# chao-ji/ldm_tf2

Measured on AMD Instinct MI355X. Metric: images/sec (256x256, 200 DDIM steps, CFG=5), higher is better.
Workload: dtype bf16

## Files before the change

### include/ldm_hip.h

```cpp
#ifndef LDM_HIP_H
#define LDM_HIP_H

#include <stddef.h>
#include <stdint.h>

#ifdef __cplusplus
extern "C" {
#endif

#define LDM_F32 0
#define LDM_BF16 1

#define LDM_OK 0
#define LDM_ERR_ARG (-1)
#define LDM_ERR_LAUNCH (-2)
#define LDM_ERR_WORKSPACE (-3)

#define LDM_ACT_NONE 0
#define LDM_ACT_GELU 1
#define LDM_ACT_GEGLU 2
#define LDM_ACT_SILU 3

int ldm_version(void);
int ldm_last_error(char* buf, int n);
// ... 21 lines not shown
  float alpha;
  int32_t no_lead_pad;
  void* ln_out;
  const float* ln_gamma;
  const float* ln_beta;
  int64_t ld_ln;
  float ln_eps;
  void* out2;
  int64_t ld2, stride2;
  int32_t n_split, rows2;
  const float* ln_cs;
  int32_t defer_reduce;
  const void* a2;
  int64_t lda2;
  int32_t Cin2;
} ldm_gemm_params;

int ldm_gemm(const ldm_gemm_params* p, void* stream);
int ldm_gemm_splits(const ldm_gemm_params* p);
int ldm_gemm_reduce(const ldm_gemm_params* p, void* stream);
int ldm_groupnorm_splitk_supported(int B, int HW, int C, int groups, int dtype);
int ldm_groupnorm_splitk_form(int B, int HW, int C, int groups, int dtype, int* form);
int ldm_groupnorm_splitk(const ldm_gemm_params* p, const float* gamma, const float* beta, void* gn_out,
                         int64_t ld_gn, int B, int HW, int groups, float eps, int silu, int store_out,
                         void* stream);
int ldm_gemm_ln_supported(int N, int dtype);
int ldm_gemm_plan(const ldm_gemm_params* p, int* tile, int* split_k);
size_t ldm_gemm_workspace_bytes(const ldm_gemm_params* p);

int ldm_conv3x3_small(const void* x, int64_t ldx, int in_dtype, const float* kernel_hwio,
                      const float* bias, void* out, int64_t ldo, int out_dtype,
                      int B, int H, int W, int Cin, int Cout, void* stream);

int ldm_groupnorm_nchunks(int B, int HW, int C);
int ldm_groupnorm_partial(const void* x, int64_t ldx, float* partial, int B, int HW, int C,
                          int groups, int nchunks, int dtype, void* stream);
int ldm_groupnorm_apply(const void* x, int64_t ldx, const float* partial, const float* gamma,
                        const float* beta, void* out, int64_t ldo, int B, int HW, int C,
                        int groups, int nchunks, float eps, int silu, int dtype, void* stream);
int ldm_groupnorm_fused_supported(int B, int HW, int C, int groups, int dtype);
int ldm_groupnorm_fused_form(int B, int HW, int C, int groups, int dtype, int* form);
int ldm_groupnorm_fused(const void* x, int64_t ldx, const float* gamma, const float* beta, void* out,
                        int64_t ldo, int B, int HW, int C, int groups, float eps, int silu, int dtype,
                        void* stream);
int ldm_layernorm(const void* x, int64_t ldx, const float* gamma, const float* beta, void* out,
                  int64_t ldo, int rows, int C, float eps, int dtype, void* stream);

int ldm_softmax_rows(const void* x, int64_t ldx, int in_dtype, void* out, int64_t ldo,
                     int out_dtype, int rows, int cols, float scale, void* stream);

int ldm_attention(const void* q, int64_t ldq, int64_t q_bs, const void* k, int64_t ldk,
                  int64_t k_bs, const void* vt, int64_t ldvt, int64_t vt_bs, void* out,
                  int64_t ldo, int64_t o_bs, int batch, int heads, int Tq, int Tk, int Sp,
                  float scale, int dtype, void* stream);

int ldm_attention_ms(const void* q, int64_t ldq, int64_t q_bs, const void* k, int64_t ldk,
                     int64_t k_bs, const void* vt, int64_t ldvt, int64_t vt_bs, void* out,
                     int64_t ldo, int64_t o_bs, int batch, int heads, int Tq, int Tk, int Sp,
                     int dtype, void* stream);

int ldm_st_tail(const void* att, int64_t lda, int K0, const void* wo, const float* bo, const void* r0,
                int64_t ldr0, const void* w1, const float* aux, const void* w2, const float* b2,
                const void* wp, const float* bp, const void* r1, int64_t ldr1, void* out, int64_t ldo,
                int M, int C, float eps, int dtype, void* stream);
int ldm_st_xtail(const void* q, int64_t ldq, int K0, const void* ctx_k, const void* ctx_vt, int Tk, int ldv, int T,
                 const void* wo, const float* bo, const void* r0, int64_t ldr0, const void* w1, const float* aux,
// ... 139 lines not shown
```

### ldm_tf2_amd/_lib.py

```python
from __future__ import annotations

import ctypes as C
import os

_HERE = os.path.dirname(os.path.abspath(__file__))
LIB_PATH = os.environ.get("LDM_HIP_LIB") or os.path.join(_HERE, "lib", "libldm_hip.so")

F32, BF16 = 0, 1
ACT_NONE, ACT_GELU, ACT_GEGLU, ACT_SILU = 0, 1, 2, 3
OK, ERR_ARG, ERR_LAUNCH, ERR_WORKSPACE = 0, -1, -2, -3
RESIZE_MODES = {"nearest": 0, "bilinear": 1, "bicubic": 2}
RESAMPLE_FILTERS = ("triangle", "cubic", "lanczos3")

c_i64, c_i32, c_f32, c_vp, c_sz = C.c_int64, C.c_int32, C.c_float, C.c_void_p, C.c_size_t
c_u32 = C.c_uint32


class GemmParams(C.Structure):
  _fields_ = [
      ("a", c_vp), ("w", c_vp), ("bias", c_vp), ("addend", c_vp), ("residual", c_vp),
      ("out", c_vp), ("workspace", c_vp), ("workspace_bytes", c_sz),
      ("lda", c_i64), ("ldr", c_i64), ("ldc_m", c_i64), ("ldc_n", c_i64),
      ("stride_a", c_i64), ("stride_w", c_i64), ("stride_c", c_i64), ("stride_r", c_i64),
      ("add_ld", c_i64),
      ("M", c_i32), ("N", c_i32), ("K", c_i32), ("batch", c_i32),
      ("add_rows", c_i32),
      ("conv", c_i32), ("B", c_i32), ("H", c_i32), ("W", c_i32), ("Cin", c_i32),
      ("OH", c_i32), ("OW", c_i32), ("stride", c_i32), ("upsample", c_i32),
      ("act", c_i32), ("dtype", c_i32), ("out_dtype", c_i32), ("split_k", c_i32),
      ("tile", c_i32), ("alpha", c_f32),
      ("no_lead_pad", c_i32),
      ("ln_out", c_vp), ("ln_gamma", c_vp), ("ln_beta", c_vp), ("ld_ln", c_i64), ("ln_eps", c_f32),
      ("out2", c_vp), ("ld2", c_i64), ("stride2", c_i64), ("n_split", c_i32), ("rows2", c_i32),
      ("ln_cs", c_vp), ("defer_reduce", c_i32),
      ("a2", c_vp), ("lda2", c_i64), ("Cin2", c_i32),
  ]


SIGNATURES = {
    "ldm_version": (c_i32, []),
    "ldm_last_error": (c_i32, [C.c_char_p, c_i32]),
    "ldm_gemm": (c_i32, [C.POINTER(GemmParams), c_vp]),
    "ldm_gemm_workspace_bytes": (c_sz, [C.POINTER(GemmParams)]),
    "ldm_gemm_splits": (c_i32, [C.POINTER(GemmParams)]),
    "ldm_gemm_reduce": (c_i32, [C.POINTER(GemmParams), c_vp]),
    "ldm_groupnorm_splitk_supported": (c_i32, [c_i32, c_i32, c_i32, c_i32, c_i32]),
    "ldm_groupnorm_splitk_form": (c_i32, [c_i32, c_i32, c_i32, c_i32, c_i32, C.POINTER(c_i32)]),
    "ldm_groupnorm_splitk": (c_i32, [C.POINTER(GemmParams), c_vp, c_vp, c_vp, c_i64, c_i32, c_i32, c_i32, c_f32,
                                     c_i32, c_i32, c_vp]),
    "ldm_conv3x3_small": (c_i32, [c_vp, c_i64, c_i32, c_vp, c_vp, c_vp, c_i64, c_i32,
                                  c_i32, c_i32, c_i32, c_i32, c_i32, c_vp]),
    "ldm_groupnorm_nchunks": (c_i32, [c_i32, c_i32, c_i32]),
    "ldm_groupnorm_partial": (c_i32, [c_vp, c_i64, c_vp, c_i32, c_i32, c_i32, c_i32, c_i32,
                                      c_i32, c_vp]),
    "ldm_groupnorm_apply": (c_i32, [c_vp, c_i64, c_vp, c_vp, c_vp, c_vp, c_i64, c_i32, c_i32,
                                    c_i32, c_i32, c_i32, c_f32, c_i32, c_i32, c_vp]),
    "ldm_layernorm": (c_i32, [c_vp, c_i64, c_vp, c_vp, c_vp, c_i64, c_i32, c_i32, c_f32,
                              c_i32, c_vp]),
    "ldm_softmax_rows": (c_i32, [c_vp, c_i64, c_i32, c_vp, c_i64, c_i32, c_i32, c_i32, c_f32,
                                 c_vp]),
    "ldm_attention": (c_i32, [c_vp, c_i64, c_i64, c_vp, c_i64, c_i64, c_vp, c_i64, c_i64,
                              c_vp, c_i64, c_i64, c_i32, c_i32, c_i32, c_i32, c_i32, c_f32,
                              c_i32, c_vp]),
    "ldm_attention_ms": (c_i32, [c_vp, c_i64, c_i64, c_vp, c_i64, c_i64, c_vp, c_i64, c_i64,
                                 c_vp, c_i64, c_i64, c_i32, c_i32, c_i32, c_i32, c_i32, c_i32, c_vp]),
    "ldm_st_tail": (c_i32, [c_vp, c_i64, c_i32, c_vp, c_vp, c_vp, c_i64, c_vp, c_vp, c_vp, c_vp, c_vp, c_vp, c_vp, c_i64,
                            c_vp, c_i64, c_i32, c_i32, c_f32, c_i32, c_vp]),
    "ldm_st_xtail": (c_i32, [c_vp, c_i64, c_i32, c_vp, c_vp, c_i32, c_i32, c_i32, c_vp, c_vp, c_vp, c_i64, c_vp, c_vp, c_vp,
                             c_vp, c_vp, c_vp, c_vp, c_i64, c_vp, c_i64, c_i32, c_i32, c_f32, c_i32, c_vp]),
    "ldm_st_block": (c_i32, [c_vp, c_i64, c_i32, c_vp, c_vp, c_vp, c_i64, c_vp, c_vp, c_vp, c_vp, c_vp, c_i32, c_i32, c_i32,
                             c_vp, c_vp, c_vp, c_vp, c_vp, c_vp, c_vp, c_vp, c_vp, c_i64, c_vp, c_i64, c_i32, c_i32, c_i32,
                             c_f32, c_i32, c_vp]),
    "ldm_ffn_geglu_supported": (c_i32, [c_i32, c_i32, c_i32]),
    "ldm_ffn_geglu": (c_i32, [c_vp, c_i64, c_vp, c_vp, c_vp, c_vp, c_vp, c_i64, c_i32, c_i32, c_f32, c_i32, c_vp]),
    "ldm_time_embedding": (c_i32, [c_vp, c_vp, c_vp, c_vp, c_i32, c_i32, c_vp]),
    "ldm_select_row": (c_i32, [c_vp, c_i64, c_i32, c_i32, c_vp, c_i32, c_vp, c_vp]),
    "ldm_gemv": (c_i32, [c_vp, c_i64, c_vp, c_vp, c_vp, c_i64, c_i32, c_i32, c_i32, c_i32,
                         c_i32, c_i32, c_vp]),
    "ldm_cfg_ddim_update": (c_i32, [c_vp, c_vp, c_vp, c_i64, c_vp, c_vp, c_vp, c_i32, c_vp, c_vp, c_i32,
                                    c_f32, c_i32, c_i32, c_i64, c_vp]),
    "ldm_cfg_ddim_update_masked": (c_i32, [c_vp, c_vp, c_vp, c_i64, c_vp, c_vp, c_vp, c_i32, c_vp, c_vp, c_i32,
                                           c_f32, c_i32, c_i32, c_i64, c_vp, c_vp, c_vp, c_i64, c_vp, c_i32, c_vp]),
    "ldm_cfg_plms_update": (c_i32, [c_vp, c_vp, c_vp, c_vp, c_vp, c_vp, c_i32, c_vp, c_vp, c_vp, c_i32, c_f32, c_i32,
                                    c_i64, c_vp, c_vp, c_vp, c_i64, c_vp, c_i32, c_vp]),
# ... 74 lines not shown
```

### ldm_tf2_amd/layout.py

```python
from __future__ import annotations

import numpy as np
import torch

ATTN_SP = (32, 48, 64, 80, 96, 160)


def padded_head(s: int) -> int:
  for sp in ATTN_SP:
    if s <= sp:
      return sp
  raise ValueError(f"head size {s} > {ATTN_SP[-1]} is not supported by the fused attention kernel")


def _dev(a, dtype, device):
  t = a if isinstance(a, torch.Tensor) else torch.from_numpy(np.ascontiguousarray(a))
  return t.to(dtype).contiguous().to(device)


def conv_kernel(k_hwio, dtype, device):
  k = torch.from_numpy(np.ascontiguousarray(k_hwio))
  cout = k.shape[3]
  return _dev(k.permute(3, 0, 1, 2).reshape(cout, -1), dtype, device)


def upsample_phase_kernel(k_hwio, dtype, device):
  k = torch.from_numpy(np.ascontiguousarray(k_hwio)).to(torch.float64)
  assert k.shape[0] == 3 and k.shape[1] == 3
  cin, cout = k.shape[2], k.shape[3]
  groups = (((0,), (1, 2)), ((0, 1), (2,)))
  out = torch.empty(4, cout, 4 * cin, dtype=torch.float64)
  for a in range(2):
    for b in range(2):
      for dy in range(2):
        for dx in range(2):
          s = sum(k[kh, kw] for kh in groups[a][dy] for kw in groups[b][dx])
          t = dy * 2 + dx
          out[2 * a + b, :, t * cin:(t + 1) * cin] = s.t()
  return _dev(out, dtype, device)


def conv_shortcut_kernel(k_hwio, k_io, dtype, device):
  k = torch.from_numpy(np.ascontiguousarray(k_hwio))
  cout = k.shape[3]
  sc = torch.from_numpy(np.ascontiguousarray(k_io)).t()
  assert sc.shape[0] == cout
  return _dev(torch.cat([k.permute(3, 0, 1, 2).reshape(cout, -1), sc], 1), dtype, device)


def dense_kernel(k_io, dtype, device):
  return _dev(torch.from_numpy(np.ascontiguousarray(k_io)).t(), dtype, device)


def split_kernel(k_dhs, sp, dtype, device):
  k = torch.from_numpy(np.ascontiguousarray(k_dhs))
  d, h, s = k.shape
# ... 92 lines not shown
```

### ldm_tf2_amd/model_runners.py

```python
from __future__ import annotations

import sys

import numpy as np
import torch

from . import ops
from ._lib import LdmHipError
from .autoencoder import AutoencoderKL, AutoencoderVQ
from .resample import check_filter, crop_box


def _tf_linspace_f32(start, stop, num):
  start, stop = np.float32(start), np.float32(stop)
  delta = np.float32((stop - start) / np.float32(num - 1))
  inner = (start + delta * np.arange(1, num - 1, dtype=np.float32)).astype(np.float32)
  return np.concatenate([[start], inner, [stop]]).astype(np.float32)


def _extract(data, t):
  return np.asarray(data).astype(np.float32)[np.asarray(t)].reshape(-1, 1, 1, 1)


def normal_latents(seed, first_index, count, shape_hwc, stream=None):
# ... 356 lines not shown
PLMS_WEIGHTS = (
    (1.,),
    (3. / 2., -1. / 2.),
    (23. / 12., -16. / 12., 5. / 12.),
    (55. / 24., -59. / 24., 37. / 24., -9. / 24.),
)
SAMPLERS = ("ddim", "plms", "deis")
MULTISTEP = ("plms", "deis")
_GL_X, _GL_W = np.polynomial.legendre.leggauss(16)


def deis_weights(lams, lam_target):
  lams = np.asarray(lams, dtype=np.float64)
  h = float(lam_target) - lams[0]
  if not h > 0.:
    raise ValueError(f"the step must raise lambda: {lams[0]} -> {lam_target}")
  nodes = (lams - lams[0]) / h
  s = 0.5 * (_GL_X + 1.)
  ex = _GL_W * np.exp(-h * s)
  den = ex.sum()
  w = np.empty(len(nodes), dtype=np.float64)
  for m in range(len(nodes)):
    basis = np.ones_like(s)
    for k in range(len(nodes)):
      if k != m:
        basis = basis * ((s - nodes[k]) / (nodes[m] - nodes[k]))
    w[m] = (ex * basis).sum() / den
  return w


class LatentDiffusionModelSampler(LatentDiffusionModel):

  def __init__(self, *args, use_graph=True, verbose=True, temb_table=True, sampler="ddim", noise_source="host",
               skip_unguided=True, **kwargs):
    super().__init__(*args, **kwargs)
    if sampler not in SAMPLERS:
      raise ValueError(f"sampler must be one of {SAMPLERS}, got {sampler!r}")
    if noise_source not in NOISE_SOURCES:
      raise ValueError(f"noise_source must be one of {NOISE_SOURCES}, got {noise_source!r}")
    self._noise_source = noise_source
    if sampler in MULTISTEP and self._eta != 0:
      raise ValueError(f"sampler={sampler!r} is deterministic: eta must be 0, got {self._eta}")
    self._sampler = sampler
    self._use_graph = use_graph
    self._use_temb_table = bool(temb_table)
    self._temb_tbl = None
    self._pre_dec = False
    self._verbose = verbose
    self._skip_unguided = bool(skip_unguided)
    self._states = {}
    self._state_key = None
    self._graph = None
    self._graph_key = None
    self._sched_graphs = {}
    self._sched_key = None
    self._gtab = None
    self._plms_tbl = None
    self._form_events = None
    self._inv_graph = None
    self._inv_graph_key = None
    self._inv_tbl = None
    self._inv_temb = None
    self.last_step_ms = None

  def _temb_kwargs(self, dec_index):
    if self._temb_tbl is None and hasattr(self._unet, "temb_table") and self._use_temb_table:
      self._temb_tbl = self._unet.temb_table(self._steps_dev).clone()
    self._pre_dec = self._temb_tbl is not None
# ... 750 lines not shown
```

### ldm_tf2_amd/ops.py

```python
from __future__ import annotations

import ctypes as C
import os
import threading

import torch

from . import _lib
from ._lib import ACT_GEGLU, ACT_GELU, ACT_NONE, ACT_SILU, BF16, F32, GemmParams, check, lib

__all__ = [
    "ACT_NONE", "ACT_GELU", "ACT_GEGLU", "ACT_SILU", "F32", "BF16", "code", "linear", "conv3x3",
    "bmm_nt", "conv3x3_small", "groupnorm", "layernorm", "softmax_rows", "attention",
    "time_embedding", "gemv", "cfg_ddim_update", "cfg_ddim_update_masked", "cfg_plms_update", "q_sample",
    "philox_u32", "normal_fill", "q_sample_rng", "cfg_ddim_update_rng", "cfg_plms_update_rng", "cfg_ms_update",
    "cfg_ms_update_rng", "cfg_sched_update", "cfg_ddim_invert_update", "window_gather", "window_fold", "window_gather_ex", "window_fold_ex", "wrap_pad", "resize_nhwc", "resample_nhwc", "post_quant", "vq_nearest", "embedding",
    "minmax_u8", "cast",
]

_TORCH_DT = {torch.float32: F32, torch.bfloat16: BF16}
_byref = C.byref
_WS = {}
_WS_BYTES = 96 << 20


def code(dtype) -> int:
  try:
    return _TORCH_DT[dtype]
  except KeyError:
    raise TypeError(f"unsupported dtype {dtype}: the HIP path stores float32 or bfloat16")


def _stream():
  return torch.cuda.current_stream().cuda_stream


def _ptr(t):
  if t is None:
    return None
  if not t.is_cuda:
    raise ValueError("the HIP path needs device tensors (there is no CPU fallback)")
  return t.data_ptr()


def _f32(t, what):
  if t is not None and t.dtype != torch.float32:
# ... 444 lines not shown
  Bt, M, K = a.shape
  shared = w.dim() == 2
  N = w.shape[-2]
  assert a.stride(-1) == 1 and w.stride(-1) == 1 and out.stride(-1) == 1
  assert w.stride(-2) == K, "weights / second operand rows must be dense"
  p = GemmParams()
  p.a, p.w, p.out = _ptr(a), _ptr(w), _ptr(out)
  p.bias = _ptr(_f32(bias, "bias"))
  p.lda = a.stride(1)
  p.stride_a = a.stride(0)
  p.stride_w = 0 if shared else w.stride(0)
  p.stride_c = out.stride(0)
  if transposed_out:
    p.ldc_m, p.ldc_n = 1, out.stride(1)
  else:
    p.ldc_m, p.ldc_n = out.stride(1), 1
  p.M, p.N, p.K, p.batch = M, N, K, Bt
  p.act, p.dtype, p.out_dtype, p.alpha = ACT_NONE, code(a.dtype), code(out.dtype), alpha
  p.tile = tile
  _gemm(p, a.device)
  return out


def conv3x3_small(x, kernel_hwio, bias, out):
  B, H, W, Cin = x.shape
  Cout = kernel_hwio.shape[-1]
  assert kernel_hwio.is_contiguous() and kernel_hwio.dtype == torch.float32
  check(lib.ldm_conv3x3_small(_ptr(x), row_ld(x), code(x.dtype), _ptr(kernel_hwio),
                              _ptr(_f32(bias, "bias")), _ptr(out), row_ld(out), code(out.dtype),
                              B, H, W, Cin, Cout, _stream()), "ldm_conv3x3_small")
  return out


def groupnorm(x, gamma, beta, out, eps, silu=False, groups=32, partial=None, fused=None, pending=None,
              store_x=True):
  B, C = x.shape[0], x.shape[-1]
  HW = x.numel() // (B * C)
  if pending is not None and not pending.done:
    same = (pending.out.data_ptr() == x.data_ptr() and tuple(pending.out.shape) == tuple(x.shape) and
            pending.out.stride() == x.stride())
    if same and lib.ldm_groupnorm_splitk_supported(B, HW, C, groups, code(x.dtype)) and row_ld(x) == pending.p.ldc_m:
      assert out.dtype == x.dtype
      check(lib.ldm_groupnorm_splitk(_byref(pending.p), _ptr(_f32(gamma, "gamma")), _ptr(_f32(beta, "beta")),
                                     _ptr(out), row_ld(out), B, HW, groups, float(eps), int(bool(silu)),
                                     int(bool(store_x)), _stream()), "ldm_groupnorm_splitk")
      pending.done = True
      _outstanding().pop(pending.ws.data_ptr(), None)
      return out
    finish(pending)
  if fused is None:
    fused = True
  if fused and lib.ldm_groupnorm_fused_supported(B, HW, C, groups, code(x.dtype)):
    assert out.dtype == x.dtype
    check(lib.ldm_groupnorm_fused(_ptr(x), row_ld(x), _ptr(_f32(gamma, "gamma")), _ptr(_f32(beta, "beta")),
                                  _ptr(out), row_ld(out), B, HW, C, groups, float(eps), int(bool(silu)),
                                  code(x.dtype), _stream()), "ldm_groupnorm_fused")
    return out
  nch = lib.ldm_groupnorm_nchunks(B, HW, C)
  if partial is None:
    partial = torch.empty(B * nch * groups * 2, dtype=torch.float32, device=x.device)
  assert partial.numel() >= B * nch * groups * 2
  dt = code(x.dtype)
  assert out.dtype == x.dtype
  check(lib.ldm_groupnorm_partial(_ptr(x), row_ld(x), _ptr(partial), B, HW, C, groups, nch, dt,
                                  _stream()), "ldm_groupnorm_partial")
  check(lib.ldm_groupnorm_apply(_ptr(x), row_ld(x), _ptr(partial), _ptr(_f32(gamma, "gamma")),
# ... 489 lines not shown
```

### ldm_tf2_amd/unet.py

```python
from __future__ import annotations

import numpy as np
import torch

from . import layout as L
from . import ops
from .weights import init_weights, unet_manifest

GN_EPS_RES = 1e-5
GN_EPS_ST = 1e-6
LN_EPS = 1e-5


class _Res:

  def __init__(self, w, p, dtype, dev, merge_shortcut=True):
    g = lambda n: w[p + "/" + n]
    self.cin, self.cout = g("conv2d_1/kernel").shape[2], g("conv2d_1/kernel").shape[3]
    self.gn1 = (L.vec(g("group_norm_1/gamma"), dev), L.vec(g("group_norm_1/beta"), dev))
    self.conv1 = (L.conv_kernel(g("conv2d_1/kernel"), dtype, dev), L.vec(g("conv2d_1/bias"), dev))
    self.temb_k, self.temb_b = g("dense/kernel"), g("dense/bias")
    self.gn2 = (L.vec(g("group_norm_2/gamma"), dev), L.vec(g("group_norm_2/beta"), dev))
    self.conv2 = self.shortcut = self.conv2_sc = None
    if (p + "/shortcut/kernel") in w and merge_shortcut:
# ... 50 lines not shown
      if self.ms:
        c2 = float(self.s) ** -0.5 * L.MS_LOG2E
        qk_scale = torch.cat([torch.full((hs,), c2), torch.ones(hs)])
        qk_ones = L.ms_ones(heads, sp, offset=hs)
        v_ones = L.ms_ones(heads, sp)
        q_scale = torch.full((hs,), c2)
        self.ms_kbias, self.ms_vbias = v_ones.to(dev), v_ones.clone().to(dev)
      v_f = L.split_kernel(w[a1 + "/value/kernel"], sp, f32, cpu)
      self.fold = dict(
          qkv1=L.ln_fold(torch.cat([qk_f, v_f], 0), lnp[0][0], lnp[0][1], None, dtype, dev,
                         row_scale=None if qk_scale is None else torch.cat([qk_scale, torch.ones(hs)]),
                         bias_extra=None if qk_ones is None else torch.cat([qk_ones, v_ones])),
          qk1=L.ln_fold(qk_f, lnp[0][0], lnp[0][1], None, dtype, dev, row_scale=qk_scale, bias_extra=qk_ones),
          v1=L.ln_fold(v_f, lnp[0][0], lnp[0][1], None, dtype, dev, bias_extra=v_ones),
          q2=L.ln_fold(L.split_kernel(w[a2 + "/query/kernel"], sp, f32, cpu), lnp[1][0], lnp[1][1], None, dtype, dev,
                       row_scale=q_scale),
          geglu=L.ln_fold(gw, lnp[2][0], lnp[2][1], gb.numpy(), dtype, dev))
    self.ffn_aux = None
    if self.fold is not None and c == 320:
      self.ffn_aux = L.ffn_aux(self.fold["geglu"][1], self.fold["geglu"][2])
    self.ctx_k = self.ctx_vt = None


class UNet:

  def __init__(self, model_channels=320, out_channels=4, num_blocks=2,
               attention_resolutions=(4, 2, 1), dropout_rate=0.1, channel_mult=(1, 2, 4, 4),
               num_heads=8, *, weights=None, dtype=torch.float32, device="cuda:0",
               context_dim=1280, init="keras", seed=2, fuse_layernorm=False, fuse_qkv=True,
               split_qkv=True, small_conv_out=False, fold_layernorm=True, fold_min_rows=2048,
               defer_reduce=True, matrix_softmax=True, gn_single_launch=True, fused_ffn=True,
               ffn_min_rows=24576, fused_tail=True, fused_xattn=True, fused_block=True,
               shared_prefix=True, merge_qkv=True, merge_qkv_max_rows=1 << 30,
               merge_shortcut=True, merge_ffproj=True, block_min_rows=12288, phase_upsample=True):
    self._fuse_ln = bool(fuse_layernorm)
    self._fuse_qkv = bool(fuse_qkv)
    self._split_qkv = dtype == torch.bfloat16 and bool(split_qkv)
    self._small_conv_out = bool(small_conv_out)
    self._fold_ln = dtype == torch.bfloat16 and bool(fold_layernorm) and not self._fuse_ln
    self._fold_min_rows = int(fold_min_rows)
    self._matrix_softmax = bool(matrix_softmax)
    self._fused_ffn = bool(fused_ffn)
    self._fused_tail = bool(fused_tail)
    self._fused_block = bool(fused_block)
    self._fused_xattn = bool(fused_xattn)
    self._block_min_rows = int(block_min_rows)
    self._ffn_min_rows = int(ffn_min_rows)
    self._gn_single = bool(gn_single_launch)
    self._defer_reduce = bool(defer_reduce)
    self._merge_ffproj = bool(merge_ffproj)
    self._merge_shortcut = bool(merge_shortcut)
    self._merge_qkv = bool(merge_qkv)
    self._merge_qkv_max_rows = int(merge_qkv_max_rows)
    self._phase_upsample = bool(phase_upsample)
    self._shared_prefix = bool(shared_prefix)
    self._ctx_sel = None
    self._pend = None
    self._model_channels = model_channels
    self._out_channels = out_channels
    self._num_blocks = num_blocks
    self._attention_resolutions = attention_resolutions
    self._dropout_rate = dropout_rate
    self._channel_mult = tuple(channel_mult)
    self._num_heads = num_heads
    self.dtype, self.device = dtype, torch.device(device)
    self.manifest = unet_manifest(model_channels, out_channels, num_blocks, self._channel_mult,
                                  num_heads, context_dim=context_dim)
    if weights is None:
      weights = init_weights(self.manifest, seed=seed, mode=init, scope="unet")
    missing = [k for k in self.manifest if k not in weights]
    if missing:
      raise KeyError(f"UNet weights missing {len(missing)} tensors, e.g. {missing[:3]}")
    self.buf = L.Buffers(self.device)
    self._ws = ops.new_workspace(self.device)
    self._compile(weights)

  def _compile(self, w):
    dt, dev, H = self.dtype, self.device, self._num_heads
    mc = self._model_channels
    self.conv_in = (L.vec(w["conv_in/kernel"], dev), L.vec(w["conv_in/bias"], dev))
    self.time1 = (L.dense_kernel(w["time_dense1/kernel"], dt, dev), L.vec(w["time_dense1/bias"], dev))
    self.time2 = (L.dense_kernel(w["time_dense2/kernel"], dt, dev), L.vec(w["time_dense2/bias"], dev))
    res_all = []

    def mk_res(p):
      r = _Res(w, p, dt, dev, merge_shortcut=self._merge_shortcut)
      res_all.append(r)
      return r

    def mk_st(p):
      return (_ST(w, p, H, dt, dev, fold_ln=self._fold_ln, matrix_softmax=self._matrix_softmax)
              if (p + "/dense1/kernel") in w else None)

    self.in_blocks, self.skip_ch, self.skip_lvl = [], [mc], [0]
    lvl, i = 0, 0
    while any(k.startswith(f"input_blocks/{i}/") for k in w):
      p = f"input_blocks/{i}"
      if (p + "/downsample/conv/kernel") in w:
        k = w[p + "/downsample/conv/kernel"]
        self.in_blocks.append(("down", L.conv_kernel(k, dt, dev), L.vec(w[p + "/downsample/conv/bias"], dev)))
        lvl += 1
        self.skip_ch.append(k.shape[3])
      else:
        r = mk_res(p + "/residual")
        self.in_blocks.append(("res", r, mk_st(p + "/spatial_transformer")))
        self.skip_ch.append(r.cout)
      self.skip_lvl.append(lvl)
      i += 1
# ... 195 lines not shown
    else:
      lo, hi = (int(v) for v in context_rows)
      assert 0 <= lo and hi <= self._ctx_rows and hi - lo == R, (context_rows, self._ctx_rows, R)
      assert not paired_rows, "paired_rows needs the whole context"
    if out is None:
      out = torch.empty(R, h, w, self._out_channels, dtype=torch.float32, device=self.device)
    if temb_table is not None:
      assert index is not None and temb_table.shape[1] == self.temb_total
      tall = self.buf.get("temb_all", (1, self.temb_total), torch.float32)
      ops.select_row(temb_table, index, tall, pre_decrement=pre_decrement)
    else:
      assert not pre_decrement
      tall = self._temb(R, t_rows, steps, index, shared_t)
    self._ctx_sel = None if context_rows is None else slice(lo, lo + R)
    pair = bool(paired_rows and self._shared_prefix and R % 2 == 0
                and self.in_blocks[0][0] == "res" and self.in_blocks[0][2] is not None)
    B_, dt = self.buf, self.dtype
    half = R // 2
    n_in, n_out = len(self.in_blocks), len(self.out_blocks)
    prev_ch = [self.mid[2].cout] + [b[0].cout for b in self.out_blocks[:-1]]
    cats = []
    for j in range(n_out):
      i = n_in - j
      lv = self.skip_lvl[i]
      cats.append(B_.get(f"cat{j}", (R, h >> lv, w >> lv, prev_ch[j] + self.skip_ch[i]), dt))
    final = B_.get("final", (R, h, w, self.out_blocks[-1][0].cout), dt)
    skip = lambda i: cats[n_in - i][..., prev_ch[n_in - i]:]
    with ops.plan_scope(R, h, dt), ops.workspace_scope(self._ws):
      self._pend = None
      self._gnp = B_.get("gn_partial", (R * 128 * 32 * 2,), torch.float32)
      try:
        if pair:
          d0 = skip(0)
          ops.conv3x3_small(x[:half], self.conv_in[0], self.conv_in[1], d0[:half])
          ops.cast(d0[:half], d0[half:])
        else:
          ops.conv3x3_small(x, self.conv_in[0], self.conv_in[1], skip(0))
        for i, blk in enumerate(self.in_blocks):
          cur, dst = skip(i), skip(i + 1)
          if blk[0] == "down":
            self._conv_deferred(cur, blk[1], dst, bias=blk[2], stride=2)
            continue
          _, r, st = blk
          if st is None:
            self._res(r, cur, tall, dst)
          elif i == 0 and pair:
            self._flush()
            with ops.plan_scope(half, h, dt):
              tmp, tmp_full = self._pair_buf("blk_r", (half,) + tuple(dst.shape[1:3]) + (r.cout,), dt, True)
              self._res(r, cur[:half], tall if tall.shape[0] == 1 else tall[:half], tmp)
              self._st(st, tmp, dst, pair=True, x_full=tmp_full)
          else:
            tmp = B_.get("blk_r", (R,) + tuple(dst.shape[1:3]) + (r.cout,), dt)
            self._res(r, cur, tall, tmp)
            self._st(st, tmp, dst)
        cur = skip(n_in)
        r1, stm, r2 = self.mid
        shp = (R,) + tuple(cur.shape[1:3]) + (r1.cout,)
        m1 = self._res(r1, cur, tall, B_.get("blk_r", shp, dt))
        m2 = self._st(stm, m1, B_.get("blk_s", shp, dt))
        self._res(r2, m2, tall, cats[0][..., :r2.cout])
        for j, (r, st, up) in enumerate(self.out_blocks):
          xin = cats[j]
          shp = (R, xin.shape[1], xin.shape[2], r.cout)
          dst = final if j + 1 == n_out else cats[j + 1][..., :r.cout]
          o = self._res(r, xin, tall, dst if st is None and up is None else B_.get("blk_r", shp, dt))
          if st is not None:
            o = self._st(st, o, dst if up is None else B_.get("blk_s", shp, dt))
          if up is not None:
            self._flush()
            if self._phase_upsample:
              ops.conv3x3_up2(o, up[0], dst, bias=up[1])
            else:
              ops.conv3x3(o, up[0], dst, bias=up[1], upsample=True)
        t0 = B_.get("gn", tuple(final.shape), dt)
        self._gn(final, self.gn_out, GN_EPS_RES, True, t0)
        if self.conv_out_mm is not None:
          ops.conv3x3(t0, self.conv_out_mm, out, bias=self.conv_out[1])
        else:
          ops.conv3x3_small(t0, self.conv_out[0], self.conv_out[1], out)
      finally:
        self._flush()
    return out

  def temb_table(self, steps):
    n = steps.numel()
    tall = self._temb(n, steps.to(torch.int32).contiguous(), None, None, False, tag="tbl")
    return tall

  def _temb(self, R, t_rows, steps, index, shared_t, tag=""):
    B_, mc = self.buf, self._model_channels
    f32 = torch.float32
    rt = 1 if (index is not None or shared_t) else R
    emb = B_.get("temb_sin" + tag, (rt, mc), f32)
    if index is not None:
      ops.time_embedding(emb, mc, steps=steps, index=index)
    else:
      ops.time_embedding(emb, mc, t_rows=t_rows)
    th = B_.get("temb_h" + tag, (rt, 4 * mc), f32)
    ops.gemv(emb, self.time1[0], self.time1[1], th, act_out=ops.ACT_SILU)
    temb = B_.get("temb" + tag, (rt, 4 * mc), f32)
    ops.gemv(th, self.time2[0], self.time2[1], temb)
    tall = B_.get("temb_all" + tag, (rt, self.temb_total), f32)
    ops.gemv(temb, self.temb_all[0], self.temb_all[1], tall, act_in=ops.ACT_SILU)
    return tall

  def __call__(self, inputs, time, context=None, y=None, training=False):
    if training:
      raise NotImplementedError("the HIP path is inference only")
    x = torch.as_tensor(inputs, dtype=torch.float32).to(self.device).contiguous()
# ... 5 lines not shown
```

Measured before the change: 9.486.

## Add MFMA kernels for UNet input and output 3x3 convolutions

```diff
diff --git a/include/ldm_hip.h b/include/ldm_hip.h
--- a/include/ldm_hip.h
+++ b/include/ldm_hip.h
@@ -77,6 +77,12 @@
                       const float* bias, void* out, int64_t ldo, int out_dtype,
                       int B, int H, int W, int Cin, int Cout, void* stream);
 
+int ldm_conv3x3_cin4(const void* x, int64_t ldx, int in_dtype, const float* kernel_hwio, const float* bias,
+                     void* out, int64_t ldo, int out_dtype, int B, int H, int W, int Cout, int dup_rows,
+                     void* stream);
+int ldm_conv3x3_cout4(const void* x, int64_t ldx, const void* packed, const float* bias, float* out,
+                      int B, int H, int W, int Cin, int Cout, void* stream);
+
 int ldm_groupnorm_nchunks(int B, int HW, int C);
 int ldm_groupnorm_partial(const void* x, int64_t ldx, float* partial, int B, int HW, int C,
                           int groups, int nchunks, int dtype, void* stream);
diff --git a/ldm_tf2_amd/_lib.py b/ldm_tf2_amd/_lib.py
--- a/ldm_tf2_amd/_lib.py
+++ b/ldm_tf2_amd/_lib.py
@@ -50,6 +50,9 @@
                                      c_i32, c_i32, c_vp]),
     "ldm_conv3x3_small": (c_i32, [c_vp, c_i64, c_i32, c_vp, c_vp, c_vp, c_i64, c_i32,
                                   c_i32, c_i32, c_i32, c_i32, c_i32, c_vp]),
+    "ldm_conv3x3_cin4": (c_i32, [c_vp, c_i64, c_i32, c_vp, c_vp, c_vp, c_i64, c_i32,
+                                 c_i32, c_i32, c_i32, c_i32, c_i32, c_vp]),
+    "ldm_conv3x3_cout4": (c_i32, [c_vp, c_i64, c_vp, c_vp, c_vp, c_i32, c_i32, c_i32, c_i32, c_i32, c_vp]),
     "ldm_groupnorm_nchunks": (c_i32, [c_i32, c_i32, c_i32]),
     "ldm_groupnorm_partial": (c_i32, [c_vp, c_i64, c_vp, c_i32, c_i32, c_i32, c_i32, c_i32,
                                       c_i32, c_vp]),
diff --git a/ldm_tf2_amd/csrc/conv_ends.hip b/ldm_tf2_amd/csrc/conv_ends.hip
--- /dev/null
+++ b/ldm_tf2_amd/csrc/conv_ends.hip
@@ -0,0 +1,262 @@
+#include "common.h"
+
+namespace {
+
+constexpr int kWaves = 4;
+
+template <typename T> __device__ __forceinline__ float ld_f32(const T* p);
+template <> __device__ __forceinline__ float ld_f32<float>(const float* p) { return *p; }
+template <> __device__ __forceinline__ float ld_f32<bf16_t>(const bf16_t* p) { return bf2f(*p); }
+
+template <typename TI, typename TO>
+__global__ __launch_bounds__(64 * kWaves) void conv_cin4_kernel(const TI* __restrict__ x, int64_t ldx,
+                                                                const float* __restrict__ w,
+                                                                const float* __restrict__ bias,
+                                                                TO* __restrict__ out, int64_t ldo, int npix, int H,
+                                                                int W, int Cout, int64_t dup_off, int tiles_per_wave) {
+  const int lane = threadIdx.x & 63, j = lane & 15, g = lane >> 4;
+  const int ncb = (Cout + 31) >> 5;
+  const int wid = blockIdx.x * kWaves + (threadIdx.x >> 6);
+  const int cb = wid % ncb, chunk = wid / ncb;
+  const int ntiles = (npix + 15) >> 4;
+  const int t0 = chunk * tiles_per_wave;
+  if (t0 >= ntiles) return;
+  const int t1 = min(t0 + tiles_per_wave, ntiles);
+
+  float wf[9][2];
+#pragma unroll
+  for (int m = 0; m < 2; ++m) {
+    const int c = cb * 32 + 8 * (j >> 2) + 4 * m + (j & 3);
+#pragma unroll
+    for (int t = 0; t < 9; ++t) wf[t][m] = c < Cout ? w[(t * 4 + g) * Cout + c] : 0.f;
+  }
+  const int c0 = cb * 32 + 8 * g;
+  const bool c_ok = c0 < Cout;
+  f32x4 b0 = {0.f, 0.f, 0.f, 0.f}, b1 = b0;
+  if (bias && c_ok) {
+    b0 = *(const f32x4*)(bias + c0);
+    b1 = *(const f32x4*)(bias + c0 + 4);
+  }
+  const int hw = H * W;
+  auto load_taps = [&](int tile, float (&xr)[9]) -> unsigned {
+    const int p = tile * 16 + j;
+    const bool p_ok = p < npix;
+    const int b = p / hw, rem = p - b * hw, y = rem / W, xx = rem - y * W;
+    unsigned mask = 0;
+#pragma unroll
+    for (int t = 0; t < 9; ++t) {
+      const int dy = t / 3 - 1, dx = t % 3 - 1;
+      const bool ok = p_ok && (unsigned)(y + dy) < (unsigned)H && (unsigned)(xx + dx) < (unsigned)W;
+      const int q = ok ? p + dy * W + dx : (p_ok ? p : 0);
+      xr[t] = ld_f32<TI>(x + (int64_t)q * ldx + g);
+      mask |= ok ? 1u << t : 0u;
+    }
+    return mask;
+  };
+  float xr[9], xn[9] = {};
+  unsigned mk = load_taps(t0, xr), mn = 0;
+  for (int tile = t0; tile < t1; ++tile) {
+    const int p = tile * 16 + j;
+    const bool p_ok = p < npix;
+    if (tile + 1 < t1) mn = load_taps(tile + 1, xn);
+    float xv[9];
+#pragma unroll
+    for (int t = 0; t < 9; ++t) xv[t] = (mk >> t) & 1u ? xr[t] : 0.f;
+    f32x4 a0 = b0, a1 = b1;
+#pragma unroll
+    for (int t = 0; t < 9; ++t) {
+      a0 = __builtin_amdgcn_mfma_f32_16x16x4f32(wf[t][0], xv[t], a0, 0, 0, 0);
+      a1 = __builtin_amdgcn_mfma_f32_16x16x4f32(wf[t][1], xv[t], a1, 0, 0, 0);
+    }
+    if constexpr (sizeof(TO) == 2) {
+      u32x4 v, s;
+      v[0] = pack_bf2(a0[0], a0[1]); v[1] = pack_bf2(a0[2], a0[3]);
+      v[2] = pack_bf2(a1[0], a1[1]); v[3] = pack_bf2(a1[2], a1[3]);
+      const int src = ((lane >> 2) + 16 * (lane & 3)) * 4;
+#pragma unroll
+      for (int k = 0; k < 4; ++k) s[k] = (uint32_t)__builtin_amdgcn_ds_bpermute(src, (int)v[k]);
+      const int ps = tile * 16 + (lane >> 2), cs = cb * 32 + 8 * (lane & 3);
+      if (ps < npix && cs < Cout) {
+        TO* op = out + (int64_t)ps * ldo + cs;
+        *(u32x4*)op = s;
+        if (dup_off) *(u32x4*)(op + dup_off) = s;
+      }
+    } else if (p_ok && c_ok) {
+      TO* op = out + (int64_t)p * ldo + c0;
+      *(f32x4*)op = a0;
+      *(f32x4*)(op + 4) = a1;
+      if (dup_off) {
+        *(f32x4*)(op + dup_off) = a0;
+        *(f32x4*)(op + dup_off + 4) = a1;
+      }
+    }
+#pragma unroll
+    for (int t = 0; t < 9; ++t) xr[t] = xn[t];
+    mk = mn;
+  }
+}
+
+constexpr int kSegPix = 18;
+constexpr int kPitch = 5;
+constexpr int kStageLoads = (3 * kSegPix * 4 + 63) / 64;
+constexpr int kStage = 6 * 256 * 4 / 16;
+static_assert(kStage >= 3 * kSegPix * kPitch, "the staged pixels must fit the wave's region");
+
+__device__ __forceinline__ int xcd_contiguous(int bid, int nwg) {
+  const int q = nwg >> 3, r = nwg & 7, xcd = bid & 7;
+  return (xcd < r ? xcd * (q + 1) : r * (q + 1) + (xcd - r) * q) + (bid >> 3);
+}
+
+__global__ __launch_bounds__(64 * kWaves) void conv_cout4_kernel(const bf16_t* __restrict__ x, int64_t ldx,
+                                                                 const bf16_t* __restrict__ wp,
+                                                                 const float* __restrict__ bias,
+                                                                 float* __restrict__ out, int npix, int H, int W,
+                                                                 int Cin, int Cout) {
+  extern __shared__ __attribute__((aligned(16))) u32x4 sw[];
+  const int KC = Cin >> 5;
+  const int nfrag = KC * 3 * 64;
+  const int lane = threadIdx.x & 63, i = lane & 15, g = lane >> 4, wave = threadIdx.x >> 6;
+  const int wg = xcd_contiguous(blockIdx.x, gridDim.x);
+  const int p0 = (wg * kWaves + wave) * 16;
+  u32x4* stage = sw + nfrag + wave * kStage;
+  const bf16_t* gsrc[kStageLoads];
+  int sdst[kStageLoads];
+#pragma unroll
+  for (int r = 0; r < kStageLoads; ++r) {
+    const int u = min(r * 64 + lane, 3 * kSegPix * 4 - 1);
+    const int pix = u >> 2, seg = pix / kSegPix, ii = pix - seg * kSegPix;
+    const int q = min(max(p0 + (seg - 1) * W - 1 + ii, 0), npix - 1);
+    gsrc[r] = x + (int64_t)q * ldx + 8 * (u & 3);
+    sdst[r] = pix * kPitch + (u & 3);
+  }
+  u32x4 xg[2][kStageLoads];
+#pragma unroll
+  for (int d = 0; d < 2; ++d)
+#pragma unroll
+    for (int r = 0; r < kStageLoads; ++r) xg[d][r] = *(const u32x4*)(gsrc[r] + min(d, KC - 1) * 32);
+  for (int i0 = 0; i0 < nfrag; i0 += 4 * 64 * kWaves) {
+    u32x4 v[4];
+#pragma unroll
+    for (int k = 0; k < 4; ++k) v[k] = ((const u32x4*)wp)[min(i0 + k * 64 * kWaves + (int)threadIdx.x, nfrag - 1)];
+#pragma unroll
+    for (int k = 0; k < 4; ++k) {
+      const int f = i0 + k * 64 * kWaves + (int)threadIdx.x;
+      if (f < nfrag) sw[f] = v[k];
+    }
+  }
+  __syncthreads();
+
+  f32x4 acc[6];
+#pragma unroll
+  for (int r = 0; r < 6; ++r) acc[r] = f32x4{0.f, 0.f, 0.f, 0.f};
+  const u32x4* wl = sw + lane;
+  const u32x4* xl = stage + i * kPitch + g;
+  const int m6 = i % 6;
+  const u32x4* xe = stage + ((m6 >> 1) * kSegPix + 16 + (m6 & 1)) * kPitch + g;
+  auto block = [&](int d, int kc, bool load) {
+#pragma unroll
+    for (int r = 0; r < kStageLoads; ++r) stage[sdst[r]] = xg[d][r];
+    if (load) {
+#pragma unroll
+      for (int r = 0; r < kStageLoads; ++r) xg[d][r] = *(const u32x4*)(gsrc[r] + (kc + 2) * 32);
+    }
+    const bf16x8 ae = __builtin_bit_cast(bf16x8, *xe);
+#pragma unroll
+    for (int kh = 0; kh < 3; ++kh) {
+      const bf16x8 wv = __builtin_bit_cast(bf16x8, wl[(kc * 3 + kh) * 64]);
+      const bf16x8 am = __builtin_bit_cast(bf16x8, xl[kh * kSegPix * kPitch]);
+      acc[kh] = __builtin_amdgcn_mfma_f32_16x16x32_bf16(am, wv, acc[kh], 0, 0, 0);
+      acc[3 + kh] = __builtin_amdgcn_mfma_f32_16x16x32_bf16(ae, wv, acc[3 + kh], 0, 0, 0);
+    }
+  };
+  int kc = 0;
+#pragma unroll 1
+  for (; kc + 3 < KC; kc += 2) {
+    block(0, kc, true);
+    block(1, kc + 1, true);
+  }
+  if (kc + 2 < KC) {
+    block(0, kc, true);
+    block(1, kc + 1, false);
+    block(0, kc + 2, false);
+  } else {
+    block(0, kc, false);
+    if (kc + 1 < KC) block(1, kc + 1, false);
+  }
+  float* yb = (float*)stage;
+  __asm__ volatile("" ::: "memory");
+#pragma unroll
+  for (int bk = 0; bk < 6; ++bk)
+#pragma unroll
+    for (int r = 0; r < 4; ++r) yb[bk * 256 + (4 * g + r) * 16 + i] = acc[bk][r];
+  __asm__ volatile("" ::: "memory");
+  const int j = lane >> 2, co = lane & 3;
+  const int p = p0 + j;
+  const bool p_ok = p < npix;
+  const int hw = H * W;
+  const int b = p / hw, rem = p - b * hw, y = rem / W, xx = rem - y * W;
+  float v = bias && co < Cout ? bias[co] : 0.f;
+#pragma unroll
+  for (int t = 0; t < 9; ++t) {
+    const int kh = t / 3, kw = t % 3;
+    const bool ok = (unsigned)(y + kh - 1) < (unsigned)H && (unsigned)(xx + kw - 1) < (unsigned)W;
+    const int ii = j + kw;
+    const int row = ii < 16 ? kh * 16 + ii : (3 + kh) * 16 + 2 * kh + ii - 16;
+    const float yv = yb[row * 16 + kw * 4 + co];
+    v += ok ? yv : 0.f;
+  }
+  if (p_ok && co < Cout) out[(int64_t)p * Cout + co] = v;
+}
+
+}
+
+extern "C" int ldm_conv3x3_cin4(const void* x, int64_t ldx, int in_dtype, const float* kernel_hwio,
+                                const float* bias, void* out, int64_t ldo, int out_dtype, int B, int H, int W,
+                                int Cout, int dup_rows, void* stream) {
+  LDM_CHECK_ARG(x && kernel_hwio && out, "ldm_conv3x3_cin4: null pointer");
+  LDM_CHECK_ARG(DT_OK(in_dtype) && DT_OK(out_dtype), "ldm_conv3x3_cin4: bad dtype");
+  LDM_CHECK_ARG(B > 0 && H > 0 && W > 0 && Cout > 0, "ldm_conv3x3_cin4: bad dims");
+  LDM_CHECK_ARG((int64_t)B * H * W < (int64_t)1 << 30, "ldm_conv3x3_cin4: more than 2^30 pixels");
+  LDM_CHECK_ARG(Cout % 8 == 0 && ldo >= Cout && ldo % 8 == 0 && ((uintptr_t)out % 16) == 0,
+                "ldm_conv3x3_cin4: Cout and ldo must be multiples of 8, out 16-byte aligned");
+  LDM_CHECK_ARG(ldx >= 4, "ldm_conv3x3_cin4: ldx < 4");
+  LDM_CHECK_ARG(!bias || ((uintptr_t)bias % 16) == 0, "ldm_conv3x3_cin4: bias must be 16-byte aligned");
+  LDM_CHECK_ARG(dup_rows == 0 || dup_rows >= B, "ldm_conv3x3_cin4: dup_rows must be 0 or >= B");
+  const int npix = B * H * W;
+  const int ncb = (Cout + 31) / 32, ntiles = (npix + 15) / 16;
+  const int64_t units = (int64_t)ntiles * ncb;
+  const int tpw = (int)(units / 4096 < 1 ? 1 : units / 4096 > 4 ? 4 : units / 4096);
+  const int64_t waves = (int64_t)((ntiles + tpw - 1) / tpw) * ncb;
+  const int64_t nwg = (waves + kWaves - 1) / kWaves;
+  LDM_CHECK_ARG(waves + kWaves < (int64_t)1 << 31, "ldm_conv3x3_cin4: grid too large");
+  const int64_t dup_off = (int64_t)dup_rows * H * W * ldo;
+  hipStream_t s = (hipStream_t)stream;
+#define LAUNCH_CIN4(TI, TO)                                                                                     \
+  hipLaunchKernelGGL((conv_cin4_kernel<TI, TO>), dim3((unsigned)nwg), dim3(64 * kWaves), 0, s, (const TI*)x, ldx, \
+                     kernel_hwio, bias, (TO*)out, ldo, npix, H, W, Cout, dup_off, tpw)
+  if (in_dtype == LDM_F32 && out_dtype == LDM_F32) LAUNCH_CIN4(float, float);
+  else if (in_dtype == LDM_F32) LAUNCH_CIN4(float, bf16_t);
+  else if (out_dtype == LDM_F32) LAUNCH_CIN4(bf16_t, float);
+  else LAUNCH_CIN4(bf16_t, bf16_t);
+#undef LAUNCH_CIN4
+  return ldm_launch_status("ldm_conv3x3_cin4");
+}
+
+extern "C" int ldm_conv3x3_cout4(const void* x, int64_t ldx, const void* packed, const float* bias, float* out,
+                                 int B, int H, int W, int Cin, int Cout, void* stream) {
+  LDM_CHECK_ARG(x && packed && out, "ldm_conv3x3_cout4: null pointer");
+  LDM_CHECK_ARG(B > 0 && H > 0 && W > 0, "ldm_conv3x3_cout4: bad dims");
+  LDM_CHECK_ARG((int64_t)B * H * W < (int64_t)1 << 30, "ldm_conv3x3_cout4: more than 2^30 pixels");
+  LDM_CHECK_ARG(Cout >= 1 && Cout <= 4, "ldm_conv3x3_cout4: Cout must be 1..4 (got %d)", Cout);
+  LDM_CHECK_ARG(Cin > 0 && Cin % 32 == 0, "ldm_conv3x3_cout4: Cin must be a multiple of 32 (got %d)", Cin);
+  LDM_CHECK_ARG(ldx >= Cin && ldx % 8 == 0 && ((uintptr_t)x % 16) == 0 && ((uintptr_t)packed % 16) == 0 &&
+                    ((uintptr_t)out % 16) == 0,
+                "ldm_conv3x3_cout4: ldx must be a multiple of 8; x, packed weights and out 16-byte aligned");
+  const size_t shm = (size_t)(Cin / 32) * 3 * 64 * 16 + (size_t)kWaves * kStage * 16;
+  LDM_CHECK_ARG(shm <= 64 * 1024, "ldm_conv3x3_cout4: Cin = %d does not fit the LDS weight image", Cin);
+  const int npix = B * H * W;
+  const int nwg = (npix + 16 * kWaves - 1) / (16 * kWaves);
+  hipLaunchKernelGGL(conv_cout4_kernel, dim3(nwg), dim3(64 * kWaves), shm, (hipStream_t)stream, (const bf16_t*)x,
+                     ldx, (const bf16_t*)packed, bias, out, npix, H, W, Cin, Cout);
+  return ldm_launch_status("ldm_conv3x3_cout4");
+}
diff --git a/ldm_tf2_amd/layout.py b/ldm_tf2_amd/layout.py
--- a/ldm_tf2_amd/layout.py
+++ b/ldm_tf2_amd/layout.py
@@ -22,6 +22,15 @@
   k = torch.from_numpy(np.ascontiguousarray(k_hwio))
   cout = k.shape[3]
   return _dev(k.permute(3, 0, 1, 2).reshape(cout, -1), dtype, device)
+
+
+def conv_cout4_kernel(k_hwio, device):
+  k = torch.from_numpy(np.ascontiguousarray(k_hwio)).to(torch.float32)
+  cin, cout = k.shape[2], k.shape[3]
+  assert k.shape[0] == 3 and k.shape[1] == 3 and cin % 32 == 0 and 1 <= cout <= 4, tuple(k.shape)
+  p = torch.zeros(cin // 32, 3, 4, 4, 4, 8, dtype=torch.float32)
+  p[:, :, :, :3, :cout, :] = k.reshape(3, 3, cin // 32, 4, 8, cout).permute(2, 0, 3, 1, 5, 4)
+  return _dev(p.reshape(cin // 32, 3, 4, 16, 8), torch.bfloat16, device)
 
 
 def upsample_phase_kernel(k_hwio, dtype, device):
diff --git a/ldm_tf2_amd/model_runners.py b/ldm_tf2_amd/model_runners.py
--- a/ldm_tf2_amd/model_runners.py
+++ b/ldm_tf2_amd/model_runners.py
@@ -412,8 +412,10 @@
 class LatentDiffusionModelSampler(LatentDiffusionModel):
 
   def __init__(self, *args, use_graph=True, verbose=True, temb_table=True, sampler="ddim", noise_source="host",
-               skip_unguided=True, **kwargs):
+               skip_unguided=True, mfma_ends=True, **kwargs):
     super().__init__(*args, **kwargs)
+    if mfma_ends and hasattr(self._unet, "use_mfma_ends"):
+      self._unet.use_mfma_ends(True)
     if sampler not in SAMPLERS:
       raise ValueError(f"sampler must be one of {SAMPLERS}, got {sampler!r}")
     if noise_source not in NOISE_SOURCES:
diff --git a/ldm_tf2_amd/ops.py b/ldm_tf2_amd/ops.py
--- a/ldm_tf2_amd/ops.py
+++ b/ldm_tf2_amd/ops.py
@@ -11,7 +11,7 @@
 
 __all__ = [
     "ACT_NONE", "ACT_GELU", "ACT_GEGLU", "ACT_SILU", "F32", "BF16", "code", "linear", "conv3x3",
-    "bmm_nt", "conv3x3_small", "groupnorm", "layernorm", "softmax_rows", "attention",
+    "bmm_nt", "conv3x3_small", "conv3x3_cin4", "conv3x3_cout4", "groupnorm", "layernorm", "softmax_rows", "attention",
     "time_embedding", "gemv", "cfg_ddim_update", "cfg_ddim_update_masked", "cfg_plms_update", "q_sample",
     "philox_u32", "normal_fill", "q_sample_rng", "cfg_ddim_update_rng", "cfg_plms_update_rng", "cfg_ms_update",
     "cfg_ms_update_rng", "cfg_sched_update", "cfg_ddim_invert_update", "window_gather", "window_fold", "window_gather_ex", "window_fold_ex", "wrap_pad", "resize_nhwc", "resample_nhwc", "post_quant", "vq_nearest", "embedding",
@@ -522,6 +522,31 @@
   return out
 
 
+def conv3x3_cin4(x, kernel_hwio, bias, out, dup_rows=0):
+  B, H, W, Cin = x.shape
+  Cout = kernel_hwio.shape[-1]
+  dup_rows = int(dup_rows)
+  assert Cin == 4 and tuple(kernel_hwio.shape) == (3, 3, 4, Cout)
+  assert kernel_hwio.is_contiguous() and kernel_hwio.dtype == torch.float32
+  assert dup_rows == 0 or dup_rows >= B, "dup_rows: the second destination lies behind the first"
+  assert tuple(out.shape) == (B + dup_rows, H, W, Cout), (tuple(out.shape), (B + dup_rows, H, W, Cout))
+  check(lib.ldm_conv3x3_cin4(_ptr(x), row_ld(x), code(x.dtype), _ptr(kernel_hwio), _ptr(_f32(bias, "bias")),
+                             _ptr(out), row_ld(out), code(out.dtype), B, H, W, Cout, dup_rows, _stream()),
+        "ldm_conv3x3_cin4")
+  return out
+
+
+def conv3x3_cout4(x, packed, bias, out):
+  B, H, W, Cin = x.shape
+  Cout = out.shape[-1]
+  assert x.dtype == torch.bfloat16 and packed.dtype == torch.bfloat16 and packed.is_contiguous()
+  assert tuple(packed.shape) == (Cin // 32, 3, 4, 16, 8) and Cin % 32 == 0, (tuple(packed.shape), Cin)
+  assert tuple(out.shape) == (B, H, W, Cout) and out.is_contiguous() and 1 <= Cout <= 4
+  check(lib.ldm_conv3x3_cout4(_ptr(x), row_ld(x), _ptr(packed), _ptr(_f32(bias, "bias")), _ptr(_f32(out, "out")),
+                              B, H, W, Cin, Cout, _stream()), "ldm_conv3x3_cout4")
+  return out
+
+
 def groupnorm(x, gamma, beta, out, eps, silu=False, groups=32, partial=None, fused=None, pending=None,
               store_x=True):
   B, C = x.shape[0], x.shape[-1]
diff --git a/ldm_tf2_amd/unet.py b/ldm_tf2_amd/unet.py
--- a/ldm_tf2_amd/unet.py
+++ b/ldm_tf2_amd/unet.py
@@ -106,7 +106,8 @@
                defer_reduce=True, matrix_softmax=True, gn_single_launch=True, fused_ffn=True,
                ffn_min_rows=24576, fused_tail=True, fused_xattn=True, fused_block=True,
                shared_prefix=True, merge_qkv=True, merge_qkv_max_rows=1 << 30,
-               merge_shortcut=True, merge_ffproj=True, block_min_rows=12288, phase_upsample=True):
+               merge_shortcut=True, merge_ffproj=True, block_min_rows=12288, phase_upsample=True,
+               mfma_ends=False):
     self._fuse_ln = bool(fuse_layernorm)
     self._fuse_qkv = bool(fuse_qkv)
     self._split_qkv = dtype == torch.bfloat16 and bool(split_qkv)
@@ -127,6 +128,8 @@
     self._merge_qkv = bool(merge_qkv)
     self._merge_qkv_max_rows = int(merge_qkv_max_rows)
     self._phase_upsample = bool(phase_upsample)
+    self._mfma_in = self._mfma_out = False
+    self.conv_out_c4 = None
     self._shared_prefix = bool(shared_prefix)
     self._ctx_sel = None
     self._pend = None
@@ -148,6 +151,16 @@
     self.buf = L.Buffers(self.device)
     self._ws = ops.new_workspace(self.device)
     self._compile(weights)
+    self.use_mfma_ends(mfma_ends)
+
+  def use_mfma_ends(self, on=True):
+    on = bool(on) and self.dtype == torch.bfloat16 and self._out_channels <= 4
+    c_last = self.out_blocks[-1][0].cout
+    self._mfma_in = on and self._model_channels % 8 == 0
+    self._mfma_out = on and c_last % 32 == 0 and c_last <= 416
+    if self._mfma_out and self.conv_out_c4 is None:
+      self.conv_out_c4 = L.conv_cout4_kernel(self.conv_out[0].cpu().numpy(), self.device)
+    return self
 
   def _compile(self, w):
     dt, dev, H = self.dtype, self.device, self._num_heads
@@ -409,8 +422,13 @@
       try:
         if pair:
           d0 = skip(0)
-          ops.conv3x3_small(x[:half], self.conv_in[0], self.conv_in[1], d0[:half])
-          ops.cast(d0[:half], d0[half:])
+          if self._mfma_in:
+            ops.conv3x3_cin4(x[:half], self.conv_in[0], self.conv_in[1], d0, dup_rows=half)
+          else:
+            ops.conv3x3_small(x[:half], self.conv_in[0], self.conv_in[1], d0[:half])
+            ops.cast(d0[:half], d0[half:])
+        elif self._mfma_in:
+          ops.conv3x3_cin4(x, self.conv_in[0], self.conv_in[1], skip(0))
         else:
           ops.conv3x3_small(x, self.conv_in[0], self.conv_in[1], skip(0))
         for i, blk in enumerate(self.in_blocks):
@@ -452,7 +470,9 @@
               ops.conv3x3(o, up[0], dst, bias=up[1], upsample=True)
         t0 = B_.get("gn", tuple(final.shape), dt)
         self._gn(final, self.gn_out, GN_EPS_RES, True, t0)
-        if self.conv_out_mm is not None:
+        if self._mfma_out:
+          ops.conv3x3_cout4(t0, self.conv_out_c4, self.conv_out[1], out)
+        elif self.conv_out_mm is not None:
           ops.conv3x3(t0, self.conv_out_mm, out, bias=self.conv_out[1])
         else:
           ops.conv3x3_small(t0, self.conv_out[0], self.conv_out[1], out)
```

New measurement: 9.528, median of 6. About the same (+0.4%).
